# lingo-db/lingo-db

Hardware: AMD Instinct MI355X
Metric: tpch_sf100_geomean_ms (lower is better)
Workload: dtype int64/int128 decimal

## Files before the change

### lingo-db_amd/csrc/ldb_core.hip

```cpp
#include "ldb_internal.h"
#include "ldb_device.h"
#include "ldb_chain.h"
#include "ldb_expand.h"
#include <algorithm>
#include <cstdlib>
#include <memory>

static thread_local char g_err[1024] = "";
void ldb_set_error(const char* fmt, ...) {
   va_list ap;
   va_start(ap, fmt);
   vsnprintf(g_err, sizeof(g_err), fmt, ap);
   va_end(ap);
}
extern "C" const char* ldb_gpu_last_error(void) { return g_err; }

#include <atomic>
#include <functional>
#include <mutex>
static std::mutex g_opt_mu;
static std::atomic<int64_t> g_option_epoch{0};
static std::unordered_map<std::string, int64_t> g_opts;
int64_t ldb_option(const char* name, int64_t dflt) {
   std::lock_guard<std::mutex> lock(g_opt_mu);
   auto it = g_opts.find(name);
   if (it != g_opts.end()) return it->second;
   std::string env = "LDB_";
   for (const char* c = name; *c; c++) env += (char) toupper((unsigned char) *c);
   int64_t v = dflt;
   if (const char* e = getenv(env.c_str())) v = atoll(e);
   g_opts[name] = v;
   return v;
}
extern "C" int32_t ldb_gpu_set_option(const char* name, int64_t value) {
   if (!name) LDB_FAIL(LDB_ERR_INVALID, "set_option: NULL name");
   static const char* known[] = {"jit", "jit_min_rows", "lazy_filter", "lazy_min_rows", "join_ordered", "join_chained", "gb_ordered", "gb_sorted", "zone_maps", "zone_min_rows", "gb_direct", "gb_wgs_per_cu", "gb_partition", "gb_partition_min_rows", "join_radix", "join_radix_min_rows", "join_radix_min_table_bytes", "join_radix_part_bytes", "probe_batch", "debug_check", "join_direct", "join_rank", "join_coarse", "dict_encode", "dict_min_rows", "comm_transport", "comm_timeout_ms", "desc_cache", "desc_cache_mb", "plan_replay", "scan_single_pass", "lazy_strings", "lazy_strings_min_rows", "gb_partition_wc", "join_radix_wc", "join_radix_lds", "gb_dense_out", "gb_partition_values", "join_pair32", "gb_dense_keys", "jit_async", "jit_threads", "jit_disk_cache", "join_all_match", "topk_short_select", "gb_fits64", "join_coarse_fine", "join_coarse_filtered", "compact_wide_tiles", "compact_max_words", "join_fuse_max_conjuncts", "join_coarse_finest", "jit_min_rows_like", "scan_split", "jit_share_compiles", "scan_strset_min_in", "scan_expand_tiles", "scan_expand_zones", "expand_direct_pct"};
   bool ok = false;
   for (const char* k : known) ok |= strcmp(k, name) == 0;
   if (!ok) LDB_FAIL(LDB_ERR_INVALID, "set_option: unknown option '%s'", name);
   std::lock_guard<std::mutex> lock(g_opt_mu);
   g_opts[name] = value;
   g_option_epoch.fetch_add(1);
   return LDB_OK;
}
extern "C" int64_t ldb_gpu_get_option(const char* name) {
   if (!name) return -1;
   std::lock_guard<std::mutex> lock(g_opt_mu);
   auto it = g_opts.find(name);
   if (it != g_opts.end()) return it->second;
   std::string env = "LDB_";
   for (const char* c = name; *c; c++) env += (char) toupper((unsigned char) *c);
   if (const char* e = getenv(env.c_str())) return atoll(e);
   return -1;
}

double ldb_host_trace_threshold() {
   static const double thr = [] {
      const char* e = getenv("LDB_HOST_TRACE");
      return e && *e ? atof(e) : -1.0;
   }();
   return thr;
}
static size_t ldb_size_class(size_t bytes) {
   if (bytes <= 256) return 256;
   const int lg = 63 - __builtin_clzll((unsigned long long) (bytes - 1));
   const size_t step = (size_t) 1 << (lg >= 3 ? lg - 3 : 0);
   return (bytes + step - 1) / step * step;
}
static void ldb_cache_release(ldb_ctx* ctx) {
   for (auto& kv : ctx->parked)
      for (void* p : kv.second) (void) hipFreeAsync(p, ctx->stream);
   ctx->parked.clear();
   ctx->cache_bytes = 0;
}
int32_t ldb_dev_alloc(ldb_ctx* ctx, void** out, size_t bytes) {
   const size_t cls = ctx->cache_on ? ldb_size_class(bytes + 16) : bytes + 16;
   if (ctx->cache_on) {
      auto it = ctx->parked.find(cls);
      if (it != ctx->parked.end() && !it->second.empty()) {
         std::pop_heap(it->second.begin(), it->second.end(), std::greater<void*>());
         *out = it->second.back();
         it->second.pop_back();
         ctx->cache_bytes -= cls;
         ctx->live[*out] = cls;
         return LDB_OK;
      }
   }
   hipError_t e;
   {
// ... 2009 lines not shown
```

### lingo-db_amd/csrc/ldb_join.hip

```cpp
#include "ldb_internal.h"
#include "ldb_join_kernel.h"
#include "ldb_jit.h"
#include <cmath>
#include "ldb_chain.h"
#include <algorithm>
#include <memory>

struct ldb_hashtable {
   ldb_ctx* ctx = nullptr;
   ldb_rel* build = nullptr;
   std::vector<ldb_colref> keys;
   uint64_t* slots = nullptr;
   uint64_t cap = 0;
   int32_t key32 = 0;
   int32_t unique = 0;
   int32_t ordered_slots = 0;
   int64_t kmin = 0, kmax = -1;
   uint64_t kmult = 0;
   uint32_t kmult32 = 0, ksh = 0;
   int32_t slot32 = 0;
   uint32_t* key_bits = nullptr;
   int32_t chained = 0;
   uint32_t* next = nullptr;
   int32_t direct = 0;
// ... 761 lines not shown
   ht->cap = std::max<uint64_t>(64, next_pow2_u64((uint64_t) build->n_rows * 2));
   h->n_rows = (uint64_t) build->n_rows;
   h->key32 = ht->key32;
   h->has_flags = 1;
   JoinBuild b{ctx, build, ht.get(), h, n_keys, build_unique};
   LDB_TRY(b.fresh_flags());
   if (ht->key32 && ldb_option("join_ordered", 1) != 0 && build->n_rows > 0) {
      LDB_TRY(b.key_range(keys));
      bool built = false;
      LDB_TRY(b.build_rank(&built));
      if (built) {
         *out = ht.release();
         return LDB_OK;
      }
   }
   LDB_TRY(b.choose_slots());
   LDB_TRY(b.insert());
   *out = ht.release();
   return LDB_OK;
}
extern "C" int32_t ldb_gpu_hashtable_release(ldb_ctx* ctx, ldb_hashtable* ht) {
   (void) ctx;
   delete ht;
   return LDB_OK;
}
extern "C" int64_t ldb_gpu_hashtable_slots(const ldb_hashtable* ht) { return ht ? (int64_t) ht->cap : -1; }
extern "C" int64_t ldb_gpu_hashtable_bytes(const ldb_hashtable* ht) { return ht ? (int64_t) ht->slot_bytes : -1; }

static int32_t make_probe_desc(ldb_hashtable* ht, ldb_rel* probe, const ldb_colref* keys, int32_t n_keys, DJoin* h, const ldb_join_residual* resid = nullptr,
                               int32_t n_resid = 0) {
   if ((size_t) n_keys != ht->keys.size()) LDB_FAIL(LDB_ERR_INVALID, "join_probe: %d probe keys vs %zu build keys", n_keys, ht->keys.size());
   memset(h, 0, sizeof(*h));
   LDB_TRY(ldb_make_dkeys(ht->build, ht->keys.data(), n_keys, &h->bkeys));
   LDB_TRY(ldb_make_dkeys(probe, keys, n_keys, &h->pkeys));
   for (int k = 0; k < n_keys; k++) {
      bool sa = h->bkeys.cols[k].type == LDB_T_UTF8, sb = h->pkeys.cols[k].type == LDB_T_UTF8;
      bool fa = h->bkeys.cols[k].type == LDB_T_FLOAT64 || h->bkeys.cols[k].type == LDB_T_FLOAT32;
      bool fb = h->pkeys.cols[k].type == LDB_T_FLOAT64 || h->pkeys.cols[k].type == LDB_T_FLOAT32;
      if (sa != sb || fa != fb) LDB_FAIL(LDB_ERR_INVALID, "join_probe: key %d type class differs between build and probe", k);
      if ((h->bkeys.cols[k].type == LDB_T_DATE32) != (h->pkeys.cols[k].type == LDB_T_DATE32)) LDB_FAIL(LDB_ERR_INVALID, "join_probe: key %d date vs non-date", k);
      bool wa = h->bkeys.cols[k].type == LDB_T_DECIMAL128 && h->bkeys.cols[k].precision >= 19;
      bool wb = h->pkeys.cols[k].type == LDB_T_DECIMAL128 && h->pkeys.cols[k].precision >= 19;
      if (wa != wb) LDB_FAIL(LDB_ERR_INVALID, "join_probe: key %d decimal width class differs (cast to a common type first)", k);
   }
   h->n_rows = (uint64_t) probe->n_rows;
   ldb_ht_layout(ht, h);
   h->rank_sorted = ht->rank_sorted;
   h->pair32 = 0;
   if (ht->pair32 && !ht->chained) {
      h->pair32 = join_pair_narrow(h->pkeys) ? 1 : 2;
   }
   h->build_unique = (ht->unique && !ht->chained) ? 1 : 0;
   h->n_ppreds = (int32_t) probe->pending.size();
   if (ht->coarse && probe->n_rows >= (1 << 22) && (probe->pending.empty() || (4u * ht->coarse_words <= 16u * 1024u && ldb_option("join_coarse_filtered", 1) != 0))) {
      h->coarse = (uint64_t) ht->coarse;
      h->coarse_words = ht->coarse_words;
      h->has_coarse = (int32_t) (32u | ht->coarse_shift);
   }
   for (size_t p = 0; p < probe->pending.size(); p++) h->ppreds[p] = probe->pending[p];
   ldb_order_preds(h->ppreds, h->n_ppreds);
   if (n_resid < 0 || n_resid > LDB_MAX_RESID || (n_resid && !resid)) LDB_FAIL(LDB_ERR_UNSUPPORTED, "join_probe: %d residual conjuncts (max %d)", n_resid, LDB_MAX_RESID);
   h->n_resid = n_resid;
   for (int32_t k = 0; k < n_resid; k++) {
      LDB_TRY(ldb_make_dcol(probe, resid[k].probe_col, &h->resid[k].pcol));
      LDB_TRY(ldb_make_dcol(ht->build, resid[k].build_col, &h->resid[k].bcol));
      const int op = resid[k].op;
      if (op < LDB_F_EQ || op > LDB_F_GTE) LDB_FAIL(LDB_ERR_INVALID, "join_probe: residual %d: comparison operator expected", k);
      for (const DCol* c : {&h->resid[k].pcol, &h->resid[k].bcol})
         if (c->type == LDB_T_UTF8 || c->type == LDB_T_FLOAT32 || c->type == LDB_T_FLOAT64) LDB_FAIL(LDB_ERR_UNSUPPORTED, "join_probe: residual %d: integer / decimal / date columns only", k);
      h->resid[k].op = op;
   }
   return LDB_OK;
}

static int32_t probe_count_impl(ldb_ctx* ctx, ldb_hashtable* ht, ldb_rel* probe, const ldb_colref* keys, int32_t n_keys, int64_t* matches, bool radix_ok, const RadixProbe* part = nullptr);
extern "C" int32_t ldb_gpu_join_probe_count(ldb_ctx* ctx, ldb_hashtable* ht, ldb_rel* probe, const ldb_colref* keys, int32_t n_keys, int64_t* matches) {
   return probe_count_impl(ctx, ht, probe, keys, n_keys, matches, true);
}
static int32_t probe_count_impl(ldb_ctx* ctx, ldb_hashtable* ht, ldb_rel* probe, const ldb_colref* keys, int32_t n_keys, int64_t* matches, bool radix_ok, const RadixProbe* part) {
   if (!ctx || !ht || !probe || !matches) LDB_FAIL(LDB_ERR_INVALID, "join_probe_count: NULL argument");
   if (radix_ok) {
      RadixProbe rp(ctx);
      LDB_TRY(radix_prepare(ctx, ht, probe, keys, n_keys, LDB_JOIN_INNER, rp));
      if (rp.rel) {
         const ldb_colref k0 = {0, 0};
         return probe_count_impl(ctx, ht, rp.rel, &k0, 1, matches, false, &rp);
      }
   }
   auto hp = std::make_unique<DJoin>();
   LDB_TRY(make_probe_desc(ht, probe, keys, n_keys, hp.get()));
   hp->kind = LDB_JOIN_INNER;
   unsigned long long* counter;
   LDB_TRY(ldb_counters(ctx, 2, (uint64_t**) &counter));
   hp->counter = (uint64_t) counter;
   LdbDesc<DJoin> d_desc(ctx);
   LDB_TRY(d_desc.upload(hp.get(), sizeof(DJoin)));
   DJoin* d = d_desc.p;
   if (probe->n_rows && part_probe_ok(ht, part, 0)) LDB_TRY(launch_part_probe(ctx, ht, part, probe->n_rows, 0, nullptr, nullptr, counter));
   else if (probe->n_rows) LDB_TRY(launch_join(ctx, hp.get(), d, ldb_grid_for(ctx, probe->n_rows, 256, 8), "k_join_probe_count", "k_join_probe_count_spec", k_join_probe_count));
   uint64_t m = 0;
   LDB_TRY(ldb_read_u64(ctx, counter + 1, &m));
   d_desc.release();
   *matches = (int64_t) m;
   return LDB_OK;
}

extern "C" int32_t ldb_gpu_join_probe(ldb_ctx* ctx, ldb_hashtable* ht, ldb_rel* probe, const ldb_colref* keys, int32_t n_keys, int32_t kind, ldb_rel** out,
                                      ldb_table** mark_out) {
   return ldb_gpu_join_probe_residual(ctx, ht, probe, keys, n_keys, kind, nullptr, 0, out, mark_out);
}
// ... 338 lines not shown
```

### lingo-db_amd/csrc/ldb_join_kernel.h

```cpp
#pragma once
#include "ldb_keys.h"

#define LDB_MAX_RESID 2
#define LDB_MAX_M2PREDS 2
struct DJoinResid {
   DCol pcol;
   DCol bcol;
   int32_t op;
   int32_t pad;
};
struct DJoin {
   uint64_t n_rows;
   uint64_t cap;
   uint64_t slots;
   uint64_t out_probe;
   uint64_t out_build;
   uint64_t out_cap;
   uint64_t counter;
   uint64_t bitmap;
   uint64_t mark;
   uint64_t mark2;
   uint64_t match;
   uint64_t flags;
   int64_t kmin, kmax;
   uint64_t kmult;
   uint32_t kmult32, ksh;
   uint64_t key_bits;
   uint64_t next;
   uint64_t coarse;
   uint32_t coarse_words, pad_c;
   int32_t key32;
   int32_t kind;
   int32_t has_bitmap, has_mark, has_flags;
   int32_t ordered_slots;
   DKeys bkeys;
   DKeys pkeys;
   int32_t n_ppreds;
   int32_t has_key_bits;
   int32_t chained;
   int32_t build_unique;
   int32_t n_resid;
   int32_t slot32;
   int32_t direct;
   int32_t rank_sorted;
   int32_t has_coarse;
   int32_t pair32;
   DJoinResid resid[LDB_MAX_RESID];
   DPred ppreds[LDB_MAX_PREDS];
   int32_t n_m2preds;
   int32_t pad_m2;
   DPred m2preds[LDB_MAX_M2PREDS];
};

extern __shared__ uint32_t ldb_join_lds[];
__device__ __forceinline__ void d_stage_coarse(const DJoin& m, const DJoin* __restrict__ d) {
   if (!m.has_coarse) return;
   const uint32_t* src = gptr<uint32_t>(d->coarse);
   for (uint32_t i = threadIdx.x; i < d->coarse_words; i += blockDim.x) ldb_join_lds[i] = src[i];
   __syncthreads();
}
__device__ __forceinline__ bool d_coarse_hit(const DJoin& m, uint32_t r) {
   const uint32_t s = (uint32_t) m.has_coarse & 31u;
   return (ldb_join_lds[r >> (s + 5u)] >> ((r >> s) & 31u)) & 1u;
}
__device__ __forceinline__ bool d_probe_pass(const DJoin& m, const DJoin* __restrict__ d, uint64_t i) {
   bool pass = true;
   const int np = m.n_ppreds;
   LDB_UNROLL
   for (int p = 0; p < np; p++)
      if (pass) pass = d_eval_pred(PV(m.ppreds[p], d->ppreds[p]), i);
   return pass;
}

#define JOIN_LONG_RUN 512
__device__ __forceinline__ uint64_t d_join_slot(const DJoin& m, const DJoin* __restrict__ d, uint64_t h, int64_t key, uint64_t mask) {
   if (m.key32 && m.ordered_slots) {
      if (m.slot32) return (uint64_t) __umulhi(((uint32_t) key - (uint32_t) d->kmin) << d->ksh, d->kmult32);
      return (((uint64_t) (key - d->kmin) * d->kmult) >> 32) & mask;
   }
   uint64_t x = h;
   x ^= x >> 33;
   x *= 0xFF51AFD7ED558CCDull;
   x ^= x >> 33;
   return x & mask;
}

__device__ __forceinline__ unsigned long long d_key_pair32(const KV& keys, uint64_t i) {
   const CV a = keys.col(0), b = keys.col(1);
   const uint32_t ka = (uint32_t) d_load_i64(a, d_phys_row(a, i)), kb = (uint32_t) d_load_i64(b, d_phys_row(b, i));
   return (unsigned long long) ka | ((unsigned long long) kb << 32);
}

__device__ __forceinline__ void join_build_body(const DJoin& m, const DJoin* __restrict__ d) {
   const uint64_t n = d->n_rows, mask = d->cap - 1;
   unsigned long long* slots = gptr_mut<unsigned long long>(d->slots);
   const KV bkeys(m.bkeys, d->bkeys);
   if (m.direct) {
      uint32_t* tab = gptr_mut<uint32_t>(d->slots);
      uint32_t* next = gptr_mut<uint32_t>(d->next);
      const CV c = bkeys.col(0);
      for (uint64_t i = blockIdx.x * (uint64_t) blockDim.x + threadIdx.x; i < n; i += (uint64_t) gridDim.x * blockDim.x) {
         const uint32_t row = d_phys_row(c, i);
         if (!d_valid(c, row)) continue;
// ... 518 lines not shown
      if (pw(m)) {
         offsets_of(m, d, 0);
         d_prefetch_keys32<U>(d, row0 + stride, n, k);
         words_at(m, d, 0);
      }
   }
   template <int P>
   __device__ __forceinline__ void step(const DJoin& m, const DJoin* __restrict__ d, uint64_t row0, uint64_t n, DPar<P>) {
      if (pw(m)) {
#pragma unroll
         for (int u = 0; u < U; u++) LDB_PIN(k[u]);
         offsets_of(m, d, 1 - P);
         d_prefetch_keys32<U>(d, row0 + 2 * stride, n, k);
         asm volatile("" : : : "memory");
         words_at(m, d, 1 - P);
#pragma unroll
         for (int u = 0; u < U; u++) LDB_PIN64(w[P][u]);
#pragma unroll
         for (int u = 0; u < U; u++) {
            if (off[P][u] == 0xFFFFFFFFu) cw[u] = 0u;
            else if (bits(m)) cw[u] = ((uint32_t) w[P][u] >> (off[P][u] & 31u)) & 1u;
            else cw[u] = m.direct == 2 ? d_rank_word(w[P][u], off[P][u]) : (uint32_t) w[P][u];
         }
      } else if (pf(m)) {
#pragma unroll
         for (int u = 0; u < U; u++) ck[u] = k[u];
         d_prefetch_keys32<U>(d, row0 + stride, n, k);
      }
   }
   __device__ __forceinline__ const uint32_t* keys(const DJoin& m) const { return pf(m) && !pw(m) ? ck : nullptr; }
   __device__ __forceinline__ const uint32_t* words(const DJoin& m) const { return pw(m) ? cw : nullptr; }
};

template <int U, typename TILE>
__device__ __forceinline__ void d_tile_loop(const DJoin& m, uint64_t first, uint64_t bound, uint64_t stride, TILE tile) {
   if (DProbePipe<U>::pw(m)) {
      uint64_t t0 = first;
      for (; t0 + stride < bound; t0 += 2 * stride) {
         tile(t0, DPar<0>{});
         tile(t0 + stride, DPar<1>{});
      }
      if (t0 < bound) tile(t0, DPar<0>{});
   } else {
      for (uint64_t t0 = first; t0 < bound; t0 += stride) tile(t0, DPar<0>{});
   }
}
__device__ __forceinline__ uint64_t d_wave_id() {
   return (uint64_t) blockIdx.x * (blockDim.x >> 6) + (uint64_t) __builtin_amdgcn_readfirstlane((int) (threadIdx.x >> 6));
}
#ifndef JOIN_BATCH
#define JOIN_BATCH 4
#endif

#define JP_U 4
template <int U>
__device__ __forceinline__ void d_pairs_of_rows(const DJoin& m, const DJoin* __restrict__ d, const uint64_t (&rows)[U], bool (&act)[U], uint32_t (&cnt)[U],
                                                const uint32_t* pre = nullptr, const uint32_t* prew = nullptr) {
   d_eval_conj_batch<U>(m.ppreds, d->ppreds, m.n_ppreds, rows, act);
   d_probe_batch<U>(m, d, rows, act, cnt, [&](int, uint32_t) { return m.kind != LDB_JOIN_SINGLE; }, pre, prew);
#pragma unroll
   for (int u = 0; u < U; u++)
      if (act[u] && m.kind != LDB_JOIN_INNER && cnt[u] == 0) cnt[u] = 1u;
}
__device__ __forceinline__ void join_probe_pairs_count_body(const DJoin& m, const DJoin* __restrict__ d) {
   const uint64_t n = d->n_rows;
   d_stage_coarse(m, d);
   const uint64_t n_chunks = (n + 63) / 64;
   const uint32_t lane = threadIdx.x & 63;
   const uint64_t wave = d_wave_id();
   const uint64_t n_waves = ((uint64_t) gridDim.x * blockDim.x) >> 6;
   uint32_t* chunk_cnt = gptr_mut<uint32_t>(d->match);
   unsigned long long total = 0;
   DProbePipe<JP_U> pipe;
   pipe.start(m, d, wave * JP_U * 64, n_waves * JP_U * 64, n);
   auto tile = [&](uint64_t w0, auto par) __attribute__((always_inline)) {
      uint64_t rows[JP_U];
      bool act[JP_U];
      uint32_t c[JP_U];
#pragma unroll
      for (int u = 0; u < JP_U; u++) {
         rows[u] = (w0 + u) * 64 + lane;
         act[u] = rows[u] < n;
      }
      pipe.step(m, d, w0 * 64, n, par);
      d_pairs_of_rows<JP_U>(m, d, rows, act, c, pipe.keys(m), pipe.words(m));
#pragma unroll
      for (int u = 0; u < JP_U; u++) {
         uint32_t s = c[u];
         for (int off = 32; off > 0; off >>= 1) s += __shfl_down(s, off);
         if (lane == 0 && w0 + u < n_chunks) chunk_cnt[w0 + u] = s;
         total += s;
      }
   };
   d_tile_loop<JP_U>(m, wave * JP_U, n_chunks, n_waves * JP_U, tile);
   if (lane == 0 && total) atomicAdd(gptr_mut<unsigned long long>(d->counter), total);
}
__device__ __forceinline__ void join_probe_pairs_body(const DJoin& m, const DJoin* __restrict__ d) {
   const uint64_t n = d->n_rows;
   d_stage_coarse(m, d);
   const uint64_t n_chunks = (n + 63) / 64;
   const uint32_t lane = threadIdx.x & 63;
   const uint64_t wave = d_wave_id();
   const uint64_t n_waves = ((uint64_t) gridDim.x * blockDim.x) >> 6;
   const uint32_t* chunk_off = gptr<uint32_t>(d->match);
   uint32_t* out_probe = gptr_mut<uint32_t>(d->out_probe);
   uint32_t* out_build = gptr_mut<uint32_t>(d->out_build);
   const uint64_t out_cap = d->out_cap;
   for (uint64_t w0 = wave * JP_U; w0 < n_chunks; w0 += n_waves * JP_U) {
      uint64_t rows[JP_U], at[JP_U];
      bool act[JP_U];
      uint32_t c[JP_U], emitted[JP_U];
#pragma unroll
      for (int u = 0; u < JP_U; u++) {
         rows[u] = (w0 + u) * 64 + lane;
         act[u] = rows[u] < n;
      }
      d_pairs_of_rows<JP_U>(m, d, rows, act, c);
#pragma unroll
      for (int u = 0; u < JP_U; u++) {
         uint32_t incl = c[u];
         for (int off = 1; off < 64; off <<= 1) {
            uint32_t up = __shfl_up(incl, off);
            if (lane >= (uint32_t) off) incl += up;
         }
         at[u] = (uint64_t) (w0 + u < n_chunks ? chunk_off[w0 + u] : 0u) + (incl - c[u]);
         emitted[u] = 0;
         act[u] = act[u] && c[u] != 0;
      }
      uint32_t again[JP_U];
      d_probe_batch<JP_U>(m, d, rows, act, again, [&](int u, uint32_t brow) {
         if (at[u] + emitted[u] < out_cap) {
            out_probe[at[u] + emitted[u]] = (uint32_t) rows[u];
            out_build[at[u] + emitted[u]] = brow;
         }
         emitted[u]++;
         return m.kind != LDB_JOIN_SINGLE;
      });
#pragma unroll
      for (int u = 0; u < JP_U; u++) {
         if (act[u] && emitted[u] == 0 && at[u] < out_cap) {
            out_probe[at[u]] = (uint32_t) rows[u];
            out_build[at[u]] = LDB_NULL_ROW;
         }
      }
   }
}

__device__ __forceinline__ void join_probe_count_body(const DJoin& m, const DJoin* __restrict__ d) {
   const uint64_t n = d->n_rows;
   d_stage_coarse(m, d);
   unsigned long long local = 0;
   const uint32_t lane = threadIdx.x & 63;
   const uint64_t wave = d_wave_id();
   const uint64_t n_waves = ((uint64_t) gridDim.x * blockDim.x) >> 6;
   const uint64_t n_tiles = (n + 64 * JOIN_BATCH - 1) / (64 * JOIN_BATCH);
   DProbePipe<JOIN_BATCH> pipe;
   pipe.start(m, d, wave * JOIN_BATCH * 64, n_waves * JOIN_BATCH * 64, n);
   auto tile = [&](uint64_t t, auto par) __attribute__((always_inline)) {
      uint64_t rows[JOIN_BATCH];
      bool act[JOIN_BATCH];
      uint32_t mt[JOIN_BATCH];
#pragma unroll
      for (int u = 0; u < JOIN_BATCH; u++) {
         rows[u] = (t * JOIN_BATCH + u) * 64 + lane;
         act[u] = rows[u] < n;
      }
      pipe.step(m, d, t * JOIN_BATCH * 64, n, par);
      d_eval_conj_batch<JOIN_BATCH>(m.ppreds, d->ppreds, m.n_ppreds, rows, act);
      d_probe_batch<JOIN_BATCH>(m, d, rows, act, mt, [](int, uint32_t) { return true; }, pipe.keys(m), pipe.words(m));
#pragma unroll
      for (int u = 0; u < JOIN_BATCH; u++) local += mt[u];
   };
   d_tile_loop<JOIN_BATCH>(m, wave, n_tiles, n_waves, tile);
   for (int off = 32; off > 0; off >>= 1) local += __shfl_down(local, off);
   if (lane == 0 && local) atomicAdd(gptr_mut<unsigned long long>(d->counter) + 1, local);
}

#define JT_BLOCK 256
#define JT_U 8
#define JT_ROWS (JT_BLOCK * JT_U)
#ifndef JT_PB
#define JT_PB 4
#endif
struct JoinTile {
   unsigned short q[JT_ROWS];
   unsigned long long bm[JT_ROWS / 64];
   uint32_t qn;
};
__device__ __forceinline__ void d_tile_filter(const DJoin& m, const DJoin* __restrict__ d, uint64_t base, uint64_t n, JoinTile& st) {
   const uint32_t t = threadIdx.x, lane = t & 63;
   if (t < JT_ROWS / 64) st.bm[t] = 0;
   if (t == 0) st.qn = 0;
   __syncthreads();
   uint64_t rows[JT_U];
   bool pass[JT_U];
#pragma unroll
   for (int u = 0; u < JT_U; u++) {
      rows[u] = base + (uint64_t) u * JT_BLOCK + t;
      pass[u] = rows[u] < n;
   }
   d_eval_conj_batch<JT_U>(m.ppreds, d->ppreds, m.n_ppreds, rows, pass);
#pragma unroll
   for (int u = 0; u < JT_U; u++) {
      const uint64_t mask = __ballot(pass[u]);
      uint32_t b = 0;
      if (mask != 0 && lane == (uint32_t) __builtin_ctzll(mask)) b = atomicAdd(&st.qn, (uint32_t) __popcll(mask));
      b = __shfl(b, mask ? __builtin_ctzll(mask) : 0);
      if (pass[u]) st.q[b + (uint32_t) __popcll(mask & ((1ull << lane) - 1ull))] = (unsigned short) (u * JT_BLOCK + t);
   }
   __syncthreads();
}
template <typename ON_MATCH, typename AFTER>
__device__ __forceinline__ void d_tile_probe(const DJoin& m, const DJoin* __restrict__ d, uint64_t base, JoinTile& st, ON_MATCH on_match, AFTER after) {
#ifdef JT_EXTRA_SYNC
   __syncthreads();
#endif
   const uint32_t qn = st.qn;
   for (uint32_t j0 = 0; j0 < qn; j0 += JT_PB * JT_BLOCK) {
      uint64_t rows[JT_PB];
      uint32_t rel[JT_PB], mt[JT_PB];
      bool act[JT_PB];
#pragma unroll
      for (int u = 0; u < JT_PB; u++) {
         const uint32_t j = j0 + (uint32_t) u * JT_BLOCK + threadIdx.x;
         act[u] = j < qn;
         rel[u] = act[u] ? st.q[j] : 0u;
// ... 62 lines not shown
__device__ __forceinline__ void d_block_count_add(const DJoin* __restrict__ d, unsigned long long local) {
   if (threadIdx.x < 64) {
      for (int off = 32; off > 0; off >>= 1) local += __shfl_down(local, off);
      if (threadIdx.x == 0 && local) atomicAdd(gptr_mut<unsigned long long>(d->counter), local);
   }
}

__device__ __forceinline__ void join_probe_unique_filtered_body(const DJoin& m, const DJoin* __restrict__ d) {
   __shared__ JoinTile st;
   const uint64_t n = d->n_rows;
   const uint64_t n_words = (n + 63) / 64, n_tiles = (n + JT_ROWS - 1) / JT_ROWS;
   uint32_t* match = gptr_mut<uint32_t>(d->match);
   unsigned long long local = 0;
   for (uint64_t tile = blockIdx.x; tile < n_tiles; tile += gridDim.x) {
      const uint64_t base = tile * JT_ROWS;
      d_tile_filter(m, d, base, n, st);
      d_tile_probe_first(m, d, base, st, [&](uint32_t r, uint32_t b) {
         if (b != LDB_NULL_ROW) {
            match[base + r] = b;
            atomicOr(&st.bm[r >> 6], 1ull << (r & 63));
         }
      });
      d_tile_flush(d, tile, n_words, st, local);
   }
   d_block_count_add(d, local);
}

#define JE_U 4
__device__ __forceinline__ void join_probe_exists_body(const DJoin& m, const DJoin* __restrict__ d) {
   const uint64_t n = d->n_rows;
   d_stage_coarse(m, d);
   if (m.n_ppreds > 0) {
      __shared__ JoinTile st;
      const uint64_t n_words = (n + 63) / 64, n_tiles = (n + JT_ROWS - 1) / JT_ROWS;
      unsigned long long local = 0;
      for (uint64_t tile = blockIdx.x; tile < n_tiles; tile += gridDim.x) {
         const uint64_t base = tile * JT_ROWS;
         d_tile_filter(m, d, base, n, st);
         d_tile_probe_first(m, d, base, st, [&](uint32_t r, uint32_t b) {
            if (m.kind == LDB_JOIN_ANTI ? b == LDB_NULL_ROW : b != LDB_NULL_ROW) atomicOr(&st.bm[r >> 6], 1ull << (r & 63));
         });
         d_tile_flush(d, tile, n_words, st, local);
      }
      d_block_count_add(d, local);
      return;
   }
   const uint64_t n_words = (n + 63) / 64;
   const uint32_t lane = threadIdx.x & 63;
   const uint64_t wave = d_wave_id();
   const uint64_t n_waves = ((uint64_t) gridDim.x * blockDim.x) >> 6;
   uint64_t* bitmap = gptr_mut<uint64_t>(d->bitmap);
   uint8_t* mark = gptr_mut<uint8_t>(d->mark);
   unsigned long long local = 0;
   DProbePipe<JE_U> pipe;
   pipe.start(m, d, wave * JE_U * 64, n_waves * JE_U * 64, n);
   auto tile = [&](uint64_t w0, auto par) __attribute__((always_inline)) {
      uint64_t rows[JE_U];
      bool act[JE_U];
      uint32_t first[JE_U];
#pragma unroll
      for (int u = 0; u < JE_U; u++) {
         rows[u] = (w0 + u) * 64 + lane;
         act[u] = rows[u] < n;
      }
      pipe.step(m, d, w0 * 64, n, par);
      d_probe_first<JE_U>(m, d, rows, act, first, pipe.keys(m), pipe.words(m));
#pragma unroll
      for (int u = 0; u < JE_U; u++) {
         const bool hit = first[u] != LDB_NULL_ROW;
         const bool keep = act[u] && (m.kind == LDB_JOIN_ANTI ? !hit : hit);
         if (m.has_mark && act[u]) mark[rows[u]] = hit ? 1 : 0;
         const uint64_t mm = __ballot(keep);
         if (lane == 0 && w0 + u < n_words) {
            bitmap[w0 + u] = mm;
            local += (unsigned long long) __popcll(mm);
         }
      }
   };
   d_tile_loop<JE_U>(m, wave * JE_U, n_words, n_waves * JE_U, tile);
   if (lane == 0 && local) atomicAdd(gptr_mut<unsigned long long>(d->counter), local);
}

__device__ __forceinline__ void join_probe_markbuild_body(const DJoin& m, const DJoin* __restrict__ d) {
   const uint64_t n = d->n_rows;
   d_stage_coarse(m, d);
   uint8_t* flags = gptr_mut<uint8_t>(d->mark);
   if (m.n_ppreds > 0) {
      __shared__ JoinTile st;
      const uint64_t n_tiles = (n + JT_ROWS - 1) / JT_ROWS;
      for (uint64_t tile = blockIdx.x; tile < n_tiles; tile += gridDim.x) {
         const uint64_t base = tile * JT_ROWS;
         d_tile_filter(m, d, base, n, st);
         d_tile_probe(
            m, d, base, st,
            [&](uint32_t, uint32_t b) {
               flags[b] = 1;
               return true;
            },
            [](uint32_t, uint32_t) {});
         __syncthreads();
      }
      return;
   }
   const uint32_t lane = threadIdx.x & 63;
   const uint64_t wave = d_wave_id();
   const uint64_t n_waves = ((uint64_t) gridDim.x * blockDim.x) >> 6;
   const uint64_t n_tiles = (n + 64 * JE_U - 1) / (64 * JE_U);
   DProbePipe<JE_U> pipe;
   pipe.start(m, d, wave * JE_U * 64, n_waves * JE_U * 64, n);
   auto tile = [&](uint64_t t, auto par) __attribute__((always_inline)) {
      uint64_t rows[JE_U];
      bool act[JE_U];
      uint32_t mt[JE_U];
#pragma unroll
      for (int u = 0; u < JE_U; u++) {
         rows[u] = (t * JE_U + u) * 64 + lane;
         act[u] = rows[u] < n;
      }
      pipe.step(m, d, t * JE_U * 64, n, par);
      d_probe_batch<JE_U>(
         m, d, rows, act, mt,
         [&](int u, uint32_t b) {
            flags[b] = 1;
            if (m.n_m2preds > 0) {
               bool also = true;
               LDB_UNROLL
               for (int p = 0; p < m.n_m2preds; p++)
                  if (also) also = d_eval_pred(PV(m.m2preds[p], d->m2preds[p]), rows[u]);
               if (also) gptr_mut<uint8_t>(d->mark2)[b] = 1;
            }
            return true;
         },
         pipe.keys(m), pipe.words(m));
   };
   d_tile_loop<JE_U>(m, wave, n_tiles, n_waves, tile);
}
__device__ __forceinline__ void join_flags_bitmap_body(const uint8_t* __restrict__ flags, uint64_t n, int anti, uint64_t* __restrict__ bitmap,
                                                       unsigned long long* __restrict__ counter, const uint8_t* __restrict__ not_flags = nullptr) {
   const uint64_t n_words = (n + 63) / 64;
   const uint32_t lane = threadIdx.x & 63;
   const uint64_t wave = d_wave_id();
   const uint64_t n_waves = ((uint64_t) gridDim.x * blockDim.x) >> 6;
   unsigned long long local = 0;
   for (uint64_t w = wave; w < n_words; w += n_waves) {
      const uint64_t i = w * 64 + lane;
      bool keep = i < n && ((flags[i] != 0) != (anti != 0));
      if (not_flags && keep) keep = not_flags[i] == 0;
      uint64_t mm = __ballot(keep);
      if (lane == 0) {
         bitmap[w] = mm;
         local += (unsigned long long) __popcll(mm);
      }
   }
   if (lane == 0 && local) atomicAdd(counter, local);
}

__device__ __forceinline__ void join_probe_unique_body(const DJoin& m, const DJoin* __restrict__ d) {
   d_stage_coarse(m, d);
   if (m.n_ppreds > 0 && m.has_bitmap) {
      join_probe_unique_filtered_body(m, d);
      return;
   }
   const uint64_t n = d->n_rows;
   const uint64_t n_words = (n + 63) / 64;
   const uint32_t lane = threadIdx.x & 63;
   const uint64_t wave = d_wave_id();
   const uint64_t n_waves = ((uint64_t) gridDim.x * blockDim.x) >> 6;
   uint64_t* bitmap = gptr_mut<uint64_t>(d->bitmap);
   uint32_t* match = gptr_mut<uint32_t>(d->match);
   unsigned long long local = 0;
   DProbePipe<JE_U> pipe;
   pipe.start(m, d, wave * JE_U * 64, n_waves * JE_U * 64, n);
   auto tile = [&](uint64_t w0, auto par) __attribute__((always_inline)) {
      uint32_t brow[JE_U];
      uint64_t rows[JE_U];
      bool act[JE_U], pass[JE_U];
#pragma unroll
      for (int u = 0; u < JE_U; u++) {
         rows[u] = (w0 + u) * 64 + lane;
         act[u] = pass[u] = rows[u] < n;
      }
      pipe.step(m, d, w0 * 64, n, par);
      d_eval_conj_batch<JE_U>(m.ppreds, d->ppreds, m.n_ppreds, rows, pass);
      d_probe_first<JE_U>(m, d, rows, pass, brow, pipe.keys(m), pipe.words(m));
#pragma unroll
      for (int u = 0; u < JE_U; u++) {
         if (act[u] && (brow[u] != LDB_NULL_ROW || !m.has_bitmap)) match[rows[u]] = brow[u];
         const uint64_t mm = __ballot(brow[u] != LDB_NULL_ROW);
         if (lane == 0 && w0 + u < n_words) {
            if (m.has_bitmap) bitmap[w0 + u] = mm;
            local += (unsigned long long) __popcll(mm);
         }
      }
   };
   d_tile_loop<JE_U>(m, wave * JE_U, n_words, n_waves * JE_U, tile);
   if (lane == 0 && local) atomicAdd(gptr_mut<unsigned long long>(d->counter), local);
}
```

Baseline: 3.482.

## Add lean dense-probe path with vectorized 4-row-per-lane key loads

Adds a specialized probe path for unfiltered, non-null, aligned 32-bit keys into direct/dense hash tables. Each lane loads four consecutive keys with one 128-bit nontemporal load, and the next tile's keys and slot words are software-pipelined. Bitmaps and counts are built with DPP row reductions, and mark/match results go out as vector stores. The existing pipe only handles the tail tile. The coarse-filter row threshold also becomes an option. This targets per-row load and ballot overhead in count, pairs, exists and unique probes, at the cost of code size and register pressure.

```diff
diff --git a/lingo-db_amd/csrc/ldb_core.hip b/lingo-db_amd/csrc/ldb_core.hip
--- a/lingo-db_amd/csrc/ldb_core.hip
+++ b/lingo-db_amd/csrc/ldb_core.hip
@@ -34,7 +34,7 @@
 }
 extern "C" int32_t ldb_gpu_set_option(const char* name, int64_t value) {
    if (!name) LDB_FAIL(LDB_ERR_INVALID, "set_option: NULL name");
-   static const char* known[] = {"jit", "jit_min_rows", "lazy_filter", "lazy_min_rows", "join_ordered", "join_chained", "gb_ordered", "gb_sorted", "zone_maps", "zone_min_rows", "gb_direct", "gb_wgs_per_cu", "gb_partition", "gb_partition_min_rows", "join_radix", "join_radix_min_rows", "join_radix_min_table_bytes", "join_radix_part_bytes", "probe_batch", "debug_check", "join_direct", "join_rank", "join_coarse", "dict_encode", "dict_min_rows", "comm_transport", "comm_timeout_ms", "desc_cache", "desc_cache_mb", "plan_replay", "scan_single_pass", "lazy_strings", "lazy_strings_min_rows", "gb_partition_wc", "join_radix_wc", "join_radix_lds", "gb_dense_out", "gb_partition_values", "join_pair32", "gb_dense_keys", "jit_async", "jit_threads", "jit_disk_cache", "join_all_match", "topk_short_select", "gb_fits64", "join_coarse_fine", "join_coarse_filtered", "compact_wide_tiles", "compact_max_words", "join_fuse_max_conjuncts", "join_coarse_finest", "jit_min_rows_like", "scan_split", "jit_share_compiles", "scan_strset_min_in", "scan_expand_tiles", "scan_expand_zones", "expand_direct_pct"};
+   static const char* known[] = {"jit", "jit_min_rows", "lazy_filter", "lazy_min_rows", "join_ordered", "join_chained", "gb_ordered", "gb_sorted", "zone_maps", "zone_min_rows", "gb_direct", "gb_wgs_per_cu", "gb_partition", "gb_partition_min_rows", "join_radix", "join_radix_min_rows", "join_radix_min_table_bytes", "join_radix_part_bytes", "probe_batch", "debug_check", "join_direct", "join_rank", "join_coarse", "dict_encode", "dict_min_rows", "comm_transport", "comm_timeout_ms", "desc_cache", "desc_cache_mb", "plan_replay", "scan_single_pass", "lazy_strings", "lazy_strings_min_rows", "gb_partition_wc", "join_radix_wc", "join_radix_lds", "gb_dense_out", "gb_partition_values", "join_pair32", "gb_dense_keys", "jit_async", "jit_threads", "jit_disk_cache", "join_all_match", "topk_short_select", "gb_fits64", "join_coarse_fine", "join_coarse_filtered", "join_coarse_min_rows", "join_dense_lean", "compact_wide_tiles", "compact_max_words", "join_fuse_max_conjuncts", "join_coarse_finest", "jit_min_rows_like", "scan_split", "jit_share_compiles", "scan_strset_min_in", "scan_expand_tiles", "scan_expand_zones", "expand_direct_pct"};
    bool ok = false;
    for (const char* k : known) ok |= strcmp(k, name) == 0;
    if (!ok) LDB_FAIL(LDB_ERR_INVALID, "set_option: unknown option '%s'", name);
diff --git a/lingo-db_amd/csrc/ldb_join.hip b/lingo-db_amd/csrc/ldb_join.hip
--- a/lingo-db_amd/csrc/ldb_join.hip
+++ b/lingo-db_amd/csrc/ldb_join.hip
@@ -837,10 +837,17 @@
    }
    h->build_unique = (ht->unique && !ht->chained) ? 1 : 0;
    h->n_ppreds = (int32_t) probe->pending.size();
-   if (ht->coarse && probe->n_rows >= (1 << 22) && (probe->pending.empty() || (4u * ht->coarse_words <= 16u * 1024u && ldb_option("join_coarse_filtered", 1) != 0))) {
+   if (ht->coarse && probe->n_rows >= ldb_option("join_coarse_min_rows", 1 << 22) && (probe->pending.empty() || (4u * ht->coarse_words <= 16u * 1024u && ldb_option("join_coarse_filtered", 1) != 0))) {
       h->coarse = (uint64_t) ht->coarse;
       h->coarse_words = ht->coarse_words;
       h->has_coarse = (int32_t) (32u | ht->coarse_shift);
+   }
+   {
+      const DCol& kc = h->pkeys.cols[0];
+      h->dense_lean = (ldb_option("join_dense_lean", 1) != 0 && h->key32 && h->n_ppreds == 0 && kc.width == 4 && kc.type != LDB_T_FLOAT32 && !kc.rowids && !kc.validity &&
+                       (kc.values & 15u) == 0 && probe->n_rows <= 0xFFFFFFFFll)
+                         ? 1
+                         : 0;
    }
    for (size_t p = 0; p < probe->pending.size(); p++) h->ppreds[p] = probe->pending[p];
    ldb_order_preds(h->ppreds, h->n_ppreds);
diff --git a/lingo-db_amd/csrc/ldb_join_kernel.h b/lingo-db_amd/csrc/ldb_join_kernel.h
--- a/lingo-db_amd/csrc/ldb_join_kernel.h
+++ b/lingo-db_amd/csrc/ldb_join_kernel.h
@@ -48,7 +48,7 @@
    DJoinResid resid[LDB_MAX_RESID];
    DPred ppreds[LDB_MAX_PREDS];
    int32_t n_m2preds;
-   int32_t pad_m2;
+   int32_t dense_lean;
    DPred m2preds[LDB_MAX_M2PREDS];
 };
 
@@ -673,6 +673,147 @@
 #define JOIN_BATCH 4
 #endif
 
+#define JL_ROWS 256u
+typedef uint32_t ldb_u32x4 __attribute__((ext_vector_type(4)));
+__device__ __forceinline__ bool d_dense_lean(const DJoin& m) {
+   return m.dense_lean != 0 && JOIN_BATCH == 4 && DProbePipe<4>::pw(m);
+}
+__device__ __forceinline__ uint32_t d_lean_row_or(uint32_t x) {
+   x |= (uint32_t) __builtin_amdgcn_update_dpp(0, (int) x, 0x111, 0xf, 0xf, true);
+   x |= (uint32_t) __builtin_amdgcn_update_dpp(0, (int) x, 0x112, 0xf, 0xf, true);
+   x |= (uint32_t) __builtin_amdgcn_update_dpp(0, (int) x, 0x114, 0xf, 0xf, true);
+   x |= (uint32_t) __builtin_amdgcn_update_dpp(0, (int) x, 0x118, 0xf, 0xf, true);
+   return x;
+}
+__device__ __forceinline__ uint32_t d_lean_row_sum(uint32_t x) {
+   x += (uint32_t) __builtin_amdgcn_update_dpp(0, (int) x, 0x111, 0xf, 0xf, true);
+   x += (uint32_t) __builtin_amdgcn_update_dpp(0, (int) x, 0x112, 0xf, 0xf, true);
+   x += (uint32_t) __builtin_amdgcn_update_dpp(0, (int) x, 0x114, 0xf, 0xf, true);
+   x += (uint32_t) __builtin_amdgcn_update_dpp(0, (int) x, 0x118, 0xf, 0xf, true);
+   return x;
+}
+__device__ __forceinline__ void d_lean_bitmap_store(uint64_t* __restrict__ bitmap, uint64_t base, uint32_t nib, uint32_t lane) {
+   const uint32_t v = nib << ((lane & 7u) * 4u);
+   const uint32_t lo = d_lean_row_or((lane & 8u) ? 0u : v), hi = d_lean_row_or((lane & 8u) ? v : 0u);
+   if ((lane & 15u) == 15u) bitmap[(base >> 6) + (lane >> 4)] = (uint64_t) lo | ((uint64_t) hi << 32);
+}
+__device__ __forceinline__ uint32_t d_uniform32(uint32_t x) { return (uint32_t) __builtin_amdgcn_readfirstlane((int) x); }
+struct DLeanPipe {
+   static __device__ __forceinline__ bool bits(const DJoin& m) { return d_exists_by_bits(m); }
+   uint32_t stride, n_full;
+   uint32_t k[4];
+   uint64_t w[2][4];
+   uint32_t off[2][4];
+   bool live[2][4];
+   uint32_t cw[4];
+   __device__ __forceinline__ void keys_at(const DJoin* __restrict__ d, uint32_t t) {
+      const uint32_t tt = t < n_full ? t : 0u;
+      const uint64_t a = d->pkeys.cols[0].values + (uint64_t) tt * (JL_ROWS * 4u);
+      const uint64_t as = (uint64_t) (uint32_t) __builtin_amdgcn_readfirstlane((int) (uint32_t) a) | ((uint64_t) (uint32_t) __builtin_amdgcn_readfirstlane((int) (uint32_t) (a >> 32)) << 32);
+      const ldb_u32x4* kt = gptr<ldb_u32x4>(as);
+      const ldb_u32x4 v = __builtin_nontemporal_load(&kt[threadIdx.x & 63u]);
+      k[0] = v.x;
+      k[1] = v.y;
+      k[2] = v.z;
+      k[3] = v.w;
+   }
+   __device__ __forceinline__ void offsets_of(const DJoin& m, const DJoin* __restrict__ d, int set) {
+      const uint32_t kmin32 = (uint32_t) d->kmin, span = (uint32_t) (d->kmax - d->kmin);
+      uint32_t r[4], fw[4];
+#pragma unroll
+      for (int j = 0; j < 4; j++) r[j] = k[j] - kmin32;
+      if (m.has_coarse) {
+         const uint32_t s = (uint32_t) m.has_coarse & 31u;
+#pragma unroll
+         for (int j = 0; j < 4; j++) fw[j] = ldb_join_lds[(r[j] < span ? r[j] : span) >> (s + 5u)];
+#pragma unroll
+         for (int j = 0; j < 4; j++) live[set][j] = (r[j] <= span) & (((fw[j] >> ((r[j] >> s) & 31u)) & 1u) != 0u);
+      } else {
+#pragma unroll
+         for (int j = 0; j < 4; j++) live[set][j] = r[j] <= span;
+      }
+#pragma unroll
+      for (int j = 0; j < 4; j++) off[set][j] = live[set][j] ? r[j] : 0u;
+   }
+   __device__ __forceinline__ void words_at(const DJoin& m, const DJoin* __restrict__ d, int set) {
+#pragma unroll
+      for (int j = 0; j < 4; j++) {
+         const uint32_t r = off[set][j];
+         if (m.direct == 2) w[set][j] = gptr<uint64_t>(d->slots)[r >> 5];
+         else if (bits(m)) w[set][j] = (uint64_t) gptr<uint32_t>(d->key_bits)[r >> 5];
+         else w[set][j] = (uint64_t) gptr<uint32_t>(d->slots)[r];
+      }
+   }
+   __device__ __forceinline__ void start(const DJoin& m, const DJoin* __restrict__ d, uint64_t wave, uint64_t n_waves, uint64_t n) {
+      stride = d_uniform32((uint32_t) n_waves);
+      n_full = d_uniform32((uint32_t) (n / JL_ROWS));
+#pragma unroll
+      for (int j = 0; j < 4; j++) {
+         cw[j] = 0;
+         w[0][j] = w[1][j] = 0;
+         off[0][j] = off[1][j] = 0;
+         live[0][j] = live[1][j] = false;
+      }
+      keys_at(d, d_uniform32((uint32_t) wave));
+      offsets_of(m, d, 0);
+      keys_at(d, d_uniform32((uint32_t) wave) + stride);
+      words_at(m, d, 0);
+   }
+   template <int P>
+   __device__ __forceinline__ void step(const DJoin& m, const DJoin* __restrict__ d, uint32_t t, DPar<P>, bool EX = false) {
+#pragma unroll
+      for (int j = 0; j < 4; j++) LDB_PIN(k[j]);
+      offsets_of(m, d, 1 - P);
+      keys_at(d, t + 2u * stride);
+      asm volatile("" : : : "memory");
+      words_at(m, d, 1 - P);
+#pragma unroll
+      for (int j = 0; j < 4; j++) LDB_PIN64(w[P][j]);
+#pragma unroll
+      for (int j = 0; j < 4; j++) {
+         uint32_t v;
+         if (bits(m) || (EX && m.direct == 2)) v = ((uint32_t) w[P][j] >> (off[P][j] & 31u)) & 1u;
+         else if (EX) v = (uint32_t) w[P][j] != 0u ? 1u : 0u;
+         else v = m.direct == 2 ? d_rank_word(w[P][j], off[P][j]) : (uint32_t) w[P][j];
+         cw[j] = live[P][j] ? v : 0u;
+      }
+   }
+};
+template <typename TILE>
+__device__ __forceinline__ void d_lean_loop(uint64_t wave, uint64_t n, uint64_t n_waves, TILE tile) {
+   const uint32_t n_full = d_uniform32((uint32_t) (n / JL_ROWS)), stride = d_uniform32((uint32_t) n_waves);
+   uint32_t t = d_uniform32((uint32_t) wave);
+   for (; t + stride < n_full; t += 2u * stride) {
+      tile(t, DPar<0>{});
+      tile(t + stride, DPar<1>{});
+   }
+   if (t < n_full) tile(t, DPar<0>{});
+}
+__device__ __forceinline__ uint64_t d_lean_rest(uint64_t n, uint64_t wave, uint64_t n_waves) {
+   const uint64_t full = n / JL_ROWS, n_tiles = (n + JL_ROWS - 1) / JL_ROWS;
+   return (full < n_tiles && (uint32_t) full % (uint32_t) n_waves == (uint32_t) wave) ? full : n_tiles;
+}
+
+template <typename EMIT>
+__device__ __forceinline__ void d_lean_resolve(const DJoin& m, const DJoin* __restrict__ d, const uint64_t (&rows)[4], const uint32_t (&cw)[4], uint32_t (&matches)[4], EMIT emit) {
+   bool live[4];
+#pragma unroll
+   for (int j = 0; j < 4; j++) {
+      matches[j] = 0;
+      live[j] = true;
+   }
+   d_direct_resolve<4>(m, d, rows, live, cw, d_exists_by_bits(m), matches, emit);
+}
+__device__ __forceinline__ void d_lean_first(const DJoin& m, const DJoin* __restrict__ d, const uint64_t (&rows)[4], const uint32_t (&cw)[4], uint32_t (&brow)[4]) {
+   uint32_t mt[4];
+#pragma unroll
+   for (int j = 0; j < 4; j++) brow[j] = LDB_NULL_ROW;
+   d_lean_resolve(m, d, rows, cw, mt, [&](int u, uint32_t b) {
+      brow[u] = b;
+      return false;
+   });
+}
+
 #define JP_U 4
 template <int U>
 __device__ __forceinline__ void d_pairs_of_rows(const DJoin& m, const DJoin* __restrict__ d, const uint64_t (&rows)[U], bool (&act)[U], uint32_t (&cnt)[U],
@@ -692,8 +833,37 @@
    const uint64_t n_waves = ((uint64_t) gridDim.x * blockDim.x) >> 6;
    uint32_t* chunk_cnt = gptr_mut<uint32_t>(d->match);
    unsigned long long total = 0;
+   uint64_t t_first = wave;
+   if (d_dense_lean(m) && n >= JL_ROWS) {
+      unsigned long long lt = 0;
+      DLeanPipe lp;
+      lp.start(m, d, wave, n_waves, n);
+      d_lean_loop(wave, n, n_waves, [&](uint32_t t, auto par) __attribute__((always_inline)) {
+         const uint64_t base = (uint64_t) t * JL_ROWS;
+         uint64_t rows[JP_U];
+         bool act[JP_U];
+         uint32_t c[JP_U];
+#pragma unroll
+         for (int j = 0; j < JP_U; j++) {
+            rows[j] = base + lane * 4u + (uint32_t) j;
+            act[j] = true;
+         }
+         lp.step(m, d, t, par);
+         d_lean_resolve(m, d, rows, lp.cw, c, [&](int, uint32_t) { return m.kind != LDB_JOIN_SINGLE; });
+#pragma unroll
+         for (int j = 0; j < JP_U; j++)
+            if (m.kind != LDB_JOIN_INNER && c[j] == 0) c[j] = 1u;
+         const uint32_t mine = c[0] + c[1] + c[2] + c[3];
+         const uint32_t s = d_lean_row_sum(mine);
+         if ((lane & 15u) == 15u) chunk_cnt[(base >> 6) + (lane >> 4)] = s;
+         lt += mine;
+      });
+      for (int off = 32; off > 0; off >>= 1) lt += __shfl_down(lt, off);
+      total += lt;
+      t_first = d_lean_rest(n, wave, n_waves);
+   }
    DProbePipe<JP_U> pipe;
-   pipe.start(m, d, wave * JP_U * 64, n_waves * JP_U * 64, n);
+   if (t_first * JP_U < n_chunks) pipe.start(m, d, t_first * JP_U * 64, n_waves * JP_U * 64, n);
    auto tile = [&](uint64_t w0, auto par) __attribute__((always_inline)) {
       uint64_t rows[JP_U];
       bool act[JP_U];
@@ -713,7 +883,7 @@
          total += s;
       }
    };
-   d_tile_loop<JP_U>(m, wave * JP_U, n_chunks, n_waves * JP_U, tile);
+   d_tile_loop<JP_U>(m, t_first * JP_U, n_chunks, n_waves * JP_U, tile);
    if (lane == 0 && total) atomicAdd(gptr_mut<unsigned long long>(d->counter), total);
 }
 __device__ __forceinline__ void join_probe_pairs_body(const DJoin& m, const DJoin* __restrict__ d) {
@@ -775,8 +945,29 @@
    const uint64_t wave = d_wave_id();
    const uint64_t n_waves = ((uint64_t) gridDim.x * blockDim.x) >> 6;
    const uint64_t n_tiles = (n + 64 * JOIN_BATCH - 1) / (64 * JOIN_BATCH);
+   uint64_t t_first = wave;
+   if (d_dense_lean(m) && n >= JL_ROWS) {
+      DLeanPipe lp;
+      lp.start(m, d, wave, n_waves, n);
+      d_lean_loop(wave, n, n_waves, [&](uint32_t t, auto par) __attribute__((always_inline)) {
+         const uint64_t base = (uint64_t) t * JL_ROWS;
+         uint64_t rows[4];
+         bool act[4];
+         uint32_t mt[4];
+#pragma unroll
+         for (int j = 0; j < 4; j++) {
+            rows[j] = base + lane * 4u + (uint32_t) j;
+            act[j] = true;
+         }
+         lp.step(m, d, t, par);
+         d_lean_resolve(m, d, rows, lp.cw, mt, [](int, uint32_t) { return true; });
+#pragma unroll
+         for (int j = 0; j < 4; j++) local += mt[j];
+      });
+      t_first = d_lean_rest(n, wave, n_waves);
+   }
    DProbePipe<JOIN_BATCH> pipe;
-   pipe.start(m, d, wave * JOIN_BATCH * 64, n_waves * JOIN_BATCH * 64, n);
+   if (t_first < n_tiles) pipe.start(m, d, t_first * JOIN_BATCH * 64, n_waves * JOIN_BATCH * 64, n);
    auto tile = [&](uint64_t t, auto par) __attribute__((always_inline)) {
       uint64_t rows[JOIN_BATCH];
       bool act[JOIN_BATCH];
@@ -792,7 +983,7 @@
 #pragma unroll
       for (int u = 0; u < JOIN_BATCH; u++) local += mt[u];
    };
-   d_tile_loop<JOIN_BATCH>(m, wave, n_tiles, n_waves, tile);
+   d_tile_loop<JOIN_BATCH>(m, t_first, n_tiles, n_waves, tile);
    for (int off = 32; off > 0; off >>= 1) local += __shfl_down(local, off);
    if (lane == 0 && local) atomicAdd(gptr_mut<unsigned long long>(d->counter) + 1, local);
 }
@@ -961,8 +1152,51 @@
    uint64_t* bitmap = gptr_mut<uint64_t>(d->bitmap);
    uint8_t* mark = gptr_mut<uint8_t>(d->mark);
    unsigned long long local = 0;
+   uint64_t t_first = wave;
+   if (d_dense_lean(m) && n >= JL_ROWS && (!m.has_mark || (d->mark & 3u) == 0)) {
+      uint32_t cnt = 0;
+      DLeanPipe lp;
+      lp.start(m, d, wave, n_waves, n);
+      d_lean_loop(wave, n, n_waves, [&](uint32_t t, auto par) __attribute__((always_inline)) {
+         const uint64_t base = (uint64_t) t * JL_ROWS;
+         uint64_t rows[JE_U];
+         bool act[JE_U];
+         uint32_t first[JE_U];
+#pragma unroll
+         for (int j = 0; j < JE_U; j++) {
+            rows[j] = base + lane * 4u + (uint32_t) j;
+            act[j] = true;
+         }
+         const bool ex = m.n_resid == 0;
+         lp.step(m, d, t, par, ex);
+         uint32_t nib = 0, hits = 0;
+         if (ex) {
+#pragma unroll
+            for (int j = 0; j < JE_U; j++) {
+               nib |= lp.cw[j] << j;
+               hits |= lp.cw[j] << (8 * j);
+            }
+         } else {
+            d_lean_first(m, d, rows, lp.cw, first);
+#pragma unroll
+            for (int j = 0; j < JE_U; j++) {
+               const bool hit = first[j] != LDB_NULL_ROW;
+               if (hit) nib |= 1u << j;
+               if (hit) hits |= 1u << (8 * j);
+            }
+         }
+         if (m.kind == LDB_JOIN_ANTI) nib ^= 15u;
+         if (m.has_mark) *reinterpret_cast<uint32_t*>(mark + base + lane * 4u) = hits;
+         d_lean_bitmap_store(bitmap, base, nib, lane);
+         cnt += (uint32_t) __popc(nib);
+      });
+      unsigned long long c64 = cnt;
+      for (int off = 32; off > 0; off >>= 1) c64 += __shfl_down(c64, off);
+      local += c64;
+      t_first = d_lean_rest(n, wave, n_waves);
+   }
    DProbePipe<JE_U> pipe;
-   pipe.start(m, d, wave * JE_U * 64, n_waves * JE_U * 64, n);
+   if (t_first * JE_U < n_words) pipe.start(m, d, t_first * JE_U * 64, n_waves * JE_U * 64, n);
    auto tile = [&](uint64_t w0, auto par) __attribute__((always_inline)) {
       uint64_t rows[JE_U];
       bool act[JE_U];
@@ -986,7 +1220,7 @@
          }
       }
    };
-   d_tile_loop<JE_U>(m, wave * JE_U, n_words, n_waves * JE_U, tile);
+   d_tile_loop<JE_U>(m, t_first * JE_U, n_words, n_waves * JE_U, tile);
    if (lane == 0 && local) atomicAdd(gptr_mut<unsigned long long>(d->counter), local);
 }
 
@@ -1078,8 +1312,45 @@
    uint64_t* bitmap = gptr_mut<uint64_t>(d->bitmap);
    uint32_t* match = gptr_mut<uint32_t>(d->match);
    unsigned long long local = 0;
+   uint64_t t_first = wave;
+   if (d_dense_lean(m) && n >= JL_ROWS && (d->match & 15u) == 0) {
+      uint32_t cnt = 0;
+      DLeanPipe lp;
+      lp.start(m, d, wave, n_waves, n);
+      d_lean_loop(wave, n, n_waves, [&](uint32_t t, auto par) __attribute__((always_inline)) {
+         const uint64_t base = (uint64_t) t * JL_ROWS;
+         uint32_t brow[JE_U];
+         uint64_t rows[JE_U];
+         bool act[JE_U];
+#pragma unroll
+         for (int j = 0; j < JE_U; j++) {
+            rows[j] = base + lane * 4u + (uint32_t) j;
+            act[j] = true;
+         }
+         lp.step(m, d, t, par);
+         d_lean_first(m, d, rows, lp.cw, brow);
+         uint32_t nib = 0;
+#pragma unroll
+         for (int j = 0; j < JE_U; j++)
+            if (brow[j] != LDB_NULL_ROW) nib |= 1u << j;
+         if (nib != 0 || !m.has_bitmap) {
+            ldb_u32x4 v;
+            v.x = brow[0];
+            v.y = brow[1];
+            v.z = brow[2];
+            v.w = brow[3];
+            *reinterpret_cast<ldb_u32x4*>(match + base + lane * 4u) = v;
+         }
+         if (m.has_bitmap) d_lean_bitmap_store(bitmap, base, nib, lane);
+         cnt += (uint32_t) __popc(nib);
+      });
+      unsigned long long c64 = cnt;
+      for (int off = 32; off > 0; off >>= 1) c64 += __shfl_down(c64, off);
+      local += c64;
+      t_first = d_lean_rest(n, wave, n_waves);
+   }
    DProbePipe<JE_U> pipe;
-   pipe.start(m, d, wave * JE_U * 64, n_waves * JE_U * 64, n);
+   if (t_first * JE_U < n_words) pipe.start(m, d, t_first * JE_U * 64, n_waves * JE_U * 64, n);
    auto tile = [&](uint64_t w0, auto par) __attribute__((always_inline)) {
       uint32_t brow[JE_U];
       uint64_t rows[JE_U];
@@ -1102,6 +1373,6 @@
          }
       }
    };
-   d_tile_loop<JE_U>(m, wave * JE_U, n_words, n_waves * JE_U, tile);
+   d_tile_loop<JE_U>(m, t_first * JE_U, n_words, n_waves * JE_U, tile);
    if (lane == 0 && local) atomicAdd(gptr_mut<unsigned long long>(d->counter), local);
 }
```

New measurement: 3.446 (median of 4 runs). No clear change (-1.0%).
